# KikeM/romtime

Hardware: AMD Instinct MI355X
Metric: snapshot-DoF/s for POD build (higher is better)
Workload: dtype f64

## Files before the change

romtime_amd/csrc/symeig.hip:

```cpp
#include "common.h"
#include "wave_ops.h"

namespace {

constexpr int TW_SMALL = 32;
constexpr int SLOT0 = 160;
constexpr int TW_LARGE = 128;
constexpr int LPR = 64;
constexpr int TT = 1024;
static_assert(LPR == 64, "row reductions use the whole-wave DPP sum");
constexpr int NMAX = 1024;
constexpr int VEC_ITERS = 2;

struct TriParams {
  const double* G;
  double* V;
  double* P;
  double* tau;
  double* d;
  double* e;
  int* flags;
  int n;
  int tw;
  int local;
  int spread;
  int xcd;
  long* counters;
};

__device__ __forceinline__ void st_wt(double* p, double v) {
  __hip_atomic_store(p, v, __ATOMIC_RELAXED, __HIP_MEMORY_SCOPE_AGENT);
}
__device__ __forceinline__ void st_xcd(double* p, double v, bool one_xcd) {
  if (one_xcd)
    __hip_atomic_store(p, v, __ATOMIC_RELAXED, __HIP_MEMORY_SCOPE_WORKGROUP);
  else
    st_wt(p, v);
}
__device__ __forceinline__ void st_slot(int* p, int v, bool one_xcd) {
  if (one_xcd)
    __hip_atomic_store(p, v, __ATOMIC_RELAXED, __HIP_MEMORY_SCOPE_WORKGROUP);
  else
    __hip_atomic_store(p, v, __ATOMIC_RELAXED, __HIP_MEMORY_SCOPE_AGENT);
}
__device__ __forceinline__ double ld_wt(const double* p) {
  return __hip_atomic_load(p, __ATOMIC_RELAXED, __HIP_MEMORY_SCOPE_AGENT);
}

__device__ __forceinline__ bool poll_slots(int* slots, int TW, int want, int* err) {
  const int lane = threadIdx.x & 63;
  const unsigned long long t0 = __builtin_amdgcn_s_memrealtime();
  for (;;) {
    int f = want;
    for (int w = lane; w < TW; w += 64) {
      const int g = __hip_atomic_load(&slots[w], __ATOMIC_RELAXED, __HIP_MEMORY_SCOPE_AGENT);
      f = g < f ? g : f;
    }
    if (__builtin_amdgcn_ballot_w64(f < want) == 0) return true;
    __builtin_amdgcn_s_sleep(1);
    if (__hip_atomic_load(err, __ATOMIC_RELAXED, __HIP_MEMORY_SCOPE_AGENT) != 0) return false;
    if (__builtin_amdgcn_s_memrealtime() - t0 > 50000000ull) {
      __hip_atomic_store(err, 1, __ATOMIC_RELAXED, __HIP_MEMORY_SCOPE_AGENT);
      return false;
    }
  }
}

__device__ __forceinline__ double block_sum(double x, double* s_red) {
  x = rtw::wave_sum(x);
  const int wid = threadIdx.x >> 6;
  __syncthreads();
  if ((threadIdx.x & 63) == 0) s_red[wid] = x;
  __syncthreads();
  double t = 0.0;
  for (int w = 0; w < TT / 64; ++w) t += s_red[w];
  return t;
}

template <int NM>
__global__ __launch_bounds__(TT) void symeig_tridiag_kernel(const TriParams p) {
  extern __shared__ __attribute__((aligned(16))) double sm[];
  __shared__ int s_ticket;
  if (p.spread) {
    if (threadIdx.x == 0) {
      const int xcc = (int)(__builtin_amdgcn_s_getreg((4 - 1) << 11 | (0 << 6) | 20) & 15u);
      s_ticket = (xcc == p.xcd) ? __hip_atomic_fetch_add(&p.flags[4], 1, __ATOMIC_RELAXED, __HIP_MEMORY_SCOPE_AGENT) : p.tw;
    }
    __syncthreads();
    if (s_ticket >= p.tw) return;
  }
  const int n = p.n, TW = p.tw, tid = threadIdx.x, wg = p.spread ? s_ticket : blockIdx.x, lane = tid & 63,
            wid = tid >> 6;
  const int RB = (n + TW - 1) / TW;
  const bool local = p.local != 0;
  const int lda = local ? n + 2 : n;
  double* A = sm;
  double* svb = sm + (size_t)RB * lda;
  double* sw = svb + 2 * n;
  double* sl = sw + n;
  double* sP = sl + n;
  __shared__ int s_abort;
  if (threadIdx.x == 0) s_abort = 0;
  constexpr int PER = NM / 64;

  for (int q = tid; q < RB * n; q += TT) {
    const int li = q / n, j = q % n, gi = li * TW + wg;
    A[(size_t)li * lda + j] = (gi < n) ? p.G[(size_t)gi * n + j] : 0.0;
  }
  __syncthreads();
  const int ty = tid / LPR, tx = tid % LPR;
  int hop = 0;

  double* L0 = p.P + (size_t)3 * n;
  __shared__ int s_one;
  if (local) {
    for (int j = tid; j < n; j += TT) sl[j] = A[j];
    if (tid == 0) {
      s_one = 0;
      atomicAdd(reinterpret_cast<unsigned long long*>(&p.counters[RT_CNT_EIG_ONE_XCD]), 1ull);
    }
    __syncthreads();
  } else {
  if (wg == 0)
    for (int j = tid; j < n; j += TT) st_wt(&L0[j], A[j]);
  if (tid == 0)
    __hip_atomic_store(&p.flags[8 + wg], (int)__builtin_amdgcn_s_getreg((4 - 1) << 11 | (0 << 6) | 20) + 1,
                       __ATOMIC_RELAXED, __HIP_MEMORY_SCOPE_AGENT);
  asm volatile("s_waitcnt vmcnt(0)" ::: "memory");
  __syncthreads();
  ++hop;
  if (wid == 0) {
    if (lane == 0) st_slot(&p.flags[SLOT0 + wg], hop, false);
    if (!poll_slots(&p.flags[SLOT0], TW, hop, &p.flags[3]) && lane == 0) s_abort = 1;
  }
  __syncthreads();
  if (s_abort) return;
  for (int j = tid; j < n; j += TT) sl[j] = ld_wt(&L0[j]);
  if (tid == 0) {
    const int mine = __hip_atomic_load(&p.flags[8], __ATOMIC_RELAXED, __HIP_MEMORY_SCOPE_AGENT);
    int same = (p.spread != 0) && (mine > 0);
    for (int w = 1; w < TW; ++w)
      same &= (__hip_atomic_load(&p.flags[8 + w], __ATOMIC_RELAXED, __HIP_MEMORY_SCOPE_AGENT) == mine);
    s_one = same;
    if (wg == 0) atomicAdd(reinterpret_cast<unsigned long long*>(&p.counters[same ? RT_CNT_EIG_ONE_XCD : RT_CNT_EIG_GENERAL_FORM]), 1ull);
  }
  __syncthreads();
  }
  const bool one_xcd = s_one != 0;

  __shared__ double s_tauv[2];
  constexpr bool MERGED = NM > 512;
  auto reflector = [&](const double (&x)[PER], int kk, int j0, int off, double diag) {
    double part = 0.0;
#pragma unroll
    for (int q = 0; q < PER; ++q)
      if (q > 0 || lane > off) part = fma(x[q], x[q], part);
    part = rtw::wave_sum(part);
    const double alpha = rtw::read_lane(x[0], off);
    double tau, beta, scale;
    if (part == 0.0) {
      tau = 0.0; beta = alpha; scale = 0.0;
    } else {
      beta = -copysign(sqrt(alpha * alpha + part), alpha);
      tau = (beta - alpha) / beta;
      scale = 1.0 / (alpha - beta);
    }
    const bool owner = (wg == kk % TW);
    double* svk = svb + (size_t)(kk & 1) * n;
#pragma unroll
    for (int q = 0; q < PER; ++q) {
      const int j = j0 + lane + 64 * q;
      const double vq = (q == 0 && lane == off) ? 1.0 : x[q] * scale;
      if (j < n && (q > 0 || lane >= off)) {
        svk[j] = vq;
        if (owner) p.V[(size_t)kk * n + j] = vq;
      }
    }
    if (lane == 0) {
      s_tauv[kk & 1] = tau;
      if (owner) {
        p.tau[kk] = tau;
        p.d[kk] = diag;
        p.e[kk] = beta;
      }
    }
  };

  if (wid == 0 && n > 2) {
    double x[PER];
#pragma unroll
    for (int q = 0; q < PER; ++q) {
      const int j = 1 + lane + 64 * q;
      x[q] = (j < n) ? sl[j] : 0.0;
    }
    reflector(x, 0, 1, 0, sl[0]);
  }
  __syncthreads();
  for (int k = 0; k + 2 < n; ++k) {
    const double* sv = svb + (size_t)(k & 1) * n;
    if constexpr (!MERGED) {
      if (k > 0) {
        if (wid == 0) {
          double x[PER];
#pragma unroll
          for (int q = 0; q < PER; ++q) {
            const int j = k + 1 + lane + 64 * q;
            x[q] = (j < n) ? sl[j] : 0.0;
          }
          reflector(x, k, k + 1, 0, sl[k]);
        }
        __syncthreads();
      }
    }
    const double tau = s_tauv[k & 1];
    double* Pk = p.P + (size_t)(k & 1) * n;
    double* Lk = p.P + (size_t)(2 + (k & 1)) * n;
    if (local) {
      const int gi = tid >> 3, sub = tid & 7;
      double acc = 0.0;
      if (tau != 0.0 && gi > k && gi < n) {
        const double* row = A + (size_t)gi * lda;
        for (int j = k + 1 + sub; j < n; j += 8) acc = fma(row[j], sv[j], acc);
      }
      acc += __shfl_xor(acc, 1);
      acc += __shfl_xor(acc, 2);
      acc += __shfl_xor(acc, 4);
      if (sub == 0 && tau != 0.0 && gi > k && gi < n) sP[gi] = tau * acc;
    } else
    for (int li = ty; li < RB; li += TT / LPR) {
      const int gi = li * TW + wg;
      if (gi > k && gi < n) {
        const double* row = A + (size_t)li * n;
        if (tau != 0.0) {
          double acc = 0.0;
          for (int j = k + 1 + tx; j < n; j += LPR) acc = fma(row[j], sv[j], acc);
          acc = rtw::wave_sum(acc);
          if (tx == 0) {
            if (local) sP[gi] = tau * acc;
            else st_xcd(&Pk[gi], tau * acc, one_xcd);
          }
        }
        if (gi == k + 1 && !local)
          for (int j = k + 1 + tx; j < n; j += LPR) st_xcd(&Lk[j], row[j], one_xcd);
      }
    }
    if (!local) asm volatile("s_waitcnt vmcnt(0)" ::: "memory");
    __syncthreads();
    ++hop;
    if (wid == 0) {
      if (lane == 0 && !local) st_slot(&p.flags[SLOT0 + wg], hop, one_xcd);
      double v[PER];
#pragma unroll
      for (int q = 0; q < PER; ++q) {
        const int j = k + 1 + lane + 64 * q;
        v[q] = (j < n) ? sv[j] : 0.0;
      }
      if (!local && !poll_slots(&p.flags[SLOT0], TW, hop, &p.flags[3])) {
        if (lane == 0) s_abort = 1;
      } else {
        double pv[PER], x[PER];
        const double* nextrow = A + (size_t)(k + 1) * lda;
#pragma unroll
        for (int q = 0; q < PER; ++q) {
          const int j = k + 1 + lane + 64 * q;
          if (local) {
            x[q] = (j < n) ? nextrow[j] : 0.0;
            pv[q] = (j < n && tau != 0.0) ? sP[j] : 0.0;
          } else {
            x[q] = (j < n) ? ld_wt(&Lk[j]) : 0.0;
            pv[q] = (j < n && tau != 0.0) ? ld_wt(&Pk[j]) : 0.0;
          }
        }
        if (tau != 0.0) {
          double dot = 0.0;
#pragma unroll
          for (int q = 0; q < PER; ++q) dot = fma(pv[q], v[q], dot);
          dot = rtw::wave_sum(dot);
          const double alpha2 = -0.5 * tau * dot;
#pragma unroll
          for (int q = 0; q < PER; ++q) pv[q] = fma(alpha2, v[q], pv[q]);
          const double w1 = rtw::first_lane(pv[0]);
#pragma unroll
          for (int q = 0; q < PER; ++q) {
            const int j = k + 1 + lane + 64 * q;
            x[q] = (j < n) ? x[q] - (pv[q] + w1 * v[q]) : 0.0;
            if (j < n) sw[j] = pv[q];
          }
        }
#pragma unroll
        for (int q = 0; q < PER; ++q) {
          const int j = k + 1 + lane + 64 * q;
          if (j < n) sl[j] = x[q];
        }
        if constexpr (MERGED)
          if (k + 3 < n) reflector(x, k + 1, k + 1, 1, rtw::first_lane(x[0]));
      }
    }
    __syncthreads();
    if (s_abort) return;
    if (tau == 0.0) continue;
    if (local) {
      const int gi = tid >> 3, sub = tid & 7;
      if (gi > k && gi < n) {
        double* row = A + (size_t)gi * lda;
        const double vi = sv[gi], wi = sw[gi];
        for (int j = k + 1 + sub; j < n; j += 8) row[j] -= vi * sw[j] + wi * sv[j];
      }
    } else
    for (int li = ty; li < RB; li += TT / LPR) {
      const int gi = li * TW + wg;
      if (gi > k && gi < n) {
        double* row = A + (size_t)li * n;
        const double vi = sv[gi], wi = sw[gi];
        for (int j = k + 1 + tx; j < n; j += LPR) row[j] -= vi * sw[j] + wi * sv[j];
      }
    }
  }
  __syncthreads();
  if (wg == (n - 2) % TW && tid == 0) {
    p.d[n - 2] = sl[n - 2];
    p.e[n - 2] = sl[n - 1];
  }
  if (wg == (n - 1) % TW && tid == 0) {
    p.d[n - 1] = A[(size_t)((n - 1) / TW) * lda + (n - 1)];
    p.e[n - 1] = 0.0;
  }
}

__device__ __forceinline__ double fast_rcp(double q) {
  const double r = __builtin_amdgcn_rcp(q);
  return fma(fma(-q, r, 1.0), r, r);
}

__device__ __forceinline__ int sturm_count(const double* d, const double* e2, int n, double x, double pivmin) {
  double q = d[0] - x;
  if (fabs(q) < pivmin) q = -pivmin;
  int c = (q < 0.0);
  for (int i = 1; i < n; ++i) {
    q = fma(-e2[i - 1], fast_rcp(q), d[i] - x);
    if (fabs(q) < pivmin) q = -pivmin;
    c += (q < 0.0);
  }
  return c;
}

__global__ void symeig_init_kernel(int* flags, double* tau, int n) {
  for (int i = threadIdx.x; i < SLOT0 + TW_LARGE; i += blockDim.x) flags[i] = 0;
  for (int i = threadIdx.x; i < n; i += blockDim.x) tau[i] = 0.0;
}

constexpr int BIS_NS = 2;
template <int NM>
__global__ __launch_bounds__(256) void symeig_bisect_kernel(const double* __restrict__ d, const double* __restrict__ e,
                                                            int n, int first, int count, double* __restrict__ lam,
                                                            const int* flags, int* status, long* counters) {
  if (blockIdx.x == 0 && threadIdx.x == 0) {
    if (status) *status = flags[3];
    if (flags[3]) atomicAdd(reinterpret_cast<unsigned long long*>(&counters[RT_CNT_EIG_TIMEOUT]), 1ull);
  }
  __shared__ double sd[NM], se2[NM];
  __shared__ int s_first[2][4];
  const int tid = threadIdx.x, lane = tid & 63, wid = tid >> 6, half = wid & 1;
  double glo = 1e300, ghi = -1e300, emax = 0.0;
  for (int i = lane; i < n; i += 64) {
    const double di = d[i], ei = (i + 1 < n) ? e[i] : 0.0, el = (i > 0) ? fabs(e[i - 1]) : 0.0;
    sd[i] = di;
    se2[i] = ei * ei;
    glo = fmin(glo, di - el - fabs(ei));
    ghi = fmax(ghi, di + el + fabs(ei));
    emax = fmax(emax, ei * ei);
  }
  glo = rtw::wave_min(glo);
  ghi = rtw::wave_max(ghi);
  emax = rtw::wave_max(emax);
  __syncthreads();
  const double tn = fmax(fabs(glo), fabs(ghi));
  double lo = glo - 2.2e-16 * tn * n - 1e-300, hi = ghi + 2.2e-16 * tn * n + 1e-300;
  const double pivmin = 2.2250738585072014e-308 * fmax(1.0, emax);
  const int j = first + min(2 * (int)blockIdx.x + (wid >> 1), count - 1);
  const int want = n - j;
  constexpr int NSH = 128 * BIS_NS;
  constexpr int NSEC = NSH + 1;
  for (int pass = 0; pass < 7; ++pass) {
    const double h = (hi - lo) / NSEC;
    const int s0 = BIS_NS * (64 * half + lane);
    const double x0 = lo + h * (s0 + 1), x1 = x0 + h;
    double q0 = sd[0] - x0, q1 = sd[0] - x1;
    if (fabs(q0) < pivmin) q0 = -pivmin;
    if (fabs(q1) < pivmin) q1 = -pivmin;
    int c0 = (q0 < 0.0), c1 = (q1 < 0.0);
    for (int i = 1; i < n; ++i) {
      const double di = sd[i], ei = se2[i - 1];
      q0 = fma(-ei, fast_rcp(q0), di - x0);
      q1 = fma(-ei, fast_rcp(q1), di - x1);
      if (fabs(q0) < pivmin) q0 = -pivmin;
      if (fabs(q1) < pivmin) q1 = -pivmin;
      c0 += (q0 < 0.0); c1 += (q1 < 0.0);
    }
    int first = NSH;
    if (c1 >= want) first = s0 + 1;
    if (c0 >= want) first = s0;
    first = rtw::wave_min_i32(first);
    if (lane == 0) s_first[pass & 1][wid] = first;
    __syncthreads();
    first = min(s_first[pass & 1][wid & 2], s_first[pass & 1][(wid & 2) + 1]);
    if (first == NSH) {
      lo = lo + h * NSH;
    } else {
      hi = lo + h * (first + 1);
      lo = lo + h * first;
    }
  }
  if (lane == 0 && half == 0) lam[j] = 0.5 * (lo + hi);
}

struct VecParams {
  const double* d;
  const double* e;
  const double* lam;
  const double* V;
  const double* tau;
  const double* C;
  double* W;
  int n, k;
};

constexpr int RBK = 4;

template <int NM>
__global__ __launch_bounds__(64) void symeig_wy_kernel(const double* __restrict__ V, int n, double* __restrict__ C) {
  constexpr int PER = NM / 64;
  const int b = blockIdx.x, lane = threadIdx.x, k0 = n - 3 - RBK * b;
  double v[RBK][PER];
#pragma unroll
  for (int u = 0; u < RBK; ++u)
#pragma unroll
    for (int q = 0; q < PER; ++q) {
      const int k = k0 - u, j = lane + 64 * q;
      v[u][q] = (k >= 0 && j > k && j < n) ? V[(size_t)k * n + j] : 0.0;
    }
  int slot = 0;
#pragma unroll
  for (int u = 1; u < RBK; ++u)
#pragma unroll
    for (int w = 0; w < u; ++w) {
      double dot = 0.0;
#pragma unroll
      for (int q = 0; q < PER; ++q) dot = fma(v[u][q], v[w][q], dot);
      dot = rtw::wave_sum(dot);
      if (lane == 0) C[6 * b + slot] = dot;
      ++slot;
    }
}

template <int NM>
__global__ __launch_bounds__(64) void symeig_vectors_kernel(const VecParams p) {
  extern __shared__ __attribute__((aligned(16))) double vsm[];
  double *dd = vsm, *ee = dd + NM, *ra = ee + NM + 8, *ub = ra + NM, *ud = ub + NM, *lm = ud + NM, *z = lm + NM,
         *y = z + NM;
  unsigned char* piv = reinterpret_cast<unsigned char*>(y + NM);
  const int n = p.n, t = blockIdx.x, lane = threadIdx.x;
  const double lambda = p.lam[t];
  double tnorm = 0.0;
  for (int i = lane; i < n; i += 64) {
    dd[i] = p.d[i] - lambda;
    ee[i] = (i + 1 < n) ? p.e[i] : 0.0;
    tnorm = fmax(tnorm, fabs(p.d[i]) + 2.0 * ((i + 1 < n) ? fabs(p.e[i]) : 0.0));
    unsigned s = 1664525u * (unsigned)(i + 1 + 7919 * (t + 1)) + 1013904223u;
    s ^= s >> 15; s *= 2246822519u; s ^= s >> 13;
    z[i] = (double)(s & 0xffffff) / 8388608.0 - 1.0;
  }
  if (lane == 0) ee[n] = 0.0;
  tnorm = rtw::wave_max(tnorm);
  const double tiny = 2.2e-16 * fmax(tnorm, 1e-300);
  __syncthreads();
  if (lane == 0) {
    double ak = dd[0], bk = ee[0];
#pragma unroll 4
    for (int k = 0; k + 1 < n; ++k) {
      const double ck = ee[k], an = dd[k + 1], t2 = ee[k + 1];
      const bool swap = fabs(ck) > fabs(ak);
      double pk = swap ? ck : ak;
      if (!swap && fabs(pk) < tiny) pk = copysign(tiny, pk == 0.0 ? 1.0 : pk);
      const double rp = fast_rcp(pk);
      const double mult = (swap ? ak : ck) * rp;
      ra[k] = rp;
      lm[k] = mult;
      piv[k] = swap ? 1 : 0;
      ub[k] = swap ? an : bk;
      ud[k] = swap ? t2 : 0.0;
      const double nd = swap ? fma(-mult, an, bk) : fma(-mult, bk, an);
      bk = swap ? -mult * t2 : t2;
      ak = nd;
    }
    ra[n - 1] = fast_rcp((fabs(ak) < tiny) ? copysign(tiny, ak == 0.0 ? 1.0 : ak) : ak);
    ub[n - 1] = 0.0;
    ud[n - 1] = 0.0;
  }
  __syncthreads();
  for (int it = 0; it < VEC_ITERS; ++it) {
    double zmax = 0.0;
    if (lane == 0) {
      double cur = z[0];
#pragma unroll 4
      for (int k = 0; k + 1 < n; ++k) {
        const double nxt = z[k + 1], ck = lm[k];
        const bool sw = piv[k] != 0;
        y[k] = sw ? nxt : cur;
        cur = sw ? fma(-ck, nxt, cur) : fma(-ck, cur, nxt);
      }
      y[n - 1] = cur;
      double z1 = 0.0, z2 = 0.0;
#pragma unroll 4
      for (int k = n - 1; k >= 0; --k) {
        const double zk = fma(-ud[k], z2, fma(-ub[k], z1, y[k])) * ra[k];
        z[k] = zk;
        zmax = fmax(zmax, fabs(zk));
        z2 = z1;
        z1 = zk;
      }
    }
    zmax = rtw::first_lane(zmax);
    __syncthreads();
    const double sc = 1.0 / fmax(zmax, 1e-300);
    for (int i = lane; i < n; i += 64) z[i] *= sc;
    __syncthreads();
  }
  double part = 0.0;
  for (int i = lane; i < n; i += 64) part += z[i] * z[i];
  part = rtw::wave_sum(part);
  const double inv = 1.0 / sqrt(part);
  for (int i = lane; i < n; i += 64) z[i] *= inv;
  __syncthreads();
  constexpr int PER = NM / 64;
  double zr[PER], vc[RBK][PER], vn[RBK][PER];
#pragma unroll
  for (int q = 0; q < PER; ++q) {
    const int j = lane + 64 * q;
    zr[q] = (j < n) ? z[j] : 0.0;
  }
  auto fetch = [&](int k, double (&dst)[PER]) {
#pragma unroll
    for (int q = 0; q < PER; ++q) {
      const int j = lane + 64 * q;
      dst[q] = (k >= 0 && j > k && j < n) ? p.V[(size_t)k * n + j] : 0.0;
    }
  };
#pragma unroll
  for (int u = 0; u < RBK; ++u) fetch(n - 3 - u, vc[u]);
  int blk = 0;
  for (int k0 = n - 3; k0 >= 0; k0 -= RBK, ++blk) {
#pragma unroll
    for (int u = 0; u < RBK; ++u) fetch(k0 - RBK - u, vn[u]);
    double tk[RBK], cc[6];
#pragma unroll
    for (int u = 0; u < RBK; ++u) tk[u] = (k0 - u >= 0) ? p.tau[k0 - u] : 0.0;
#pragma unroll
    for (int q = 0; q < 6; ++q) cc[q] = p.C[6 * blk + q];
    double a[RBK];
#pragma unroll
    for (int u = 0; u < RBK; ++u) {
      double dot = 0.0;
#pragma unroll
      for (int q = 0; q < PER; ++q) dot = fma(vc[u][q], zr[q], dot);
      a[u] = dot;
    }
#pragma unroll
    for (int u = 0; u < RBK; ++u) a[u] = rtw::wave_sum(a[u]);
    const double s0 = tk[0] * a[0];
    const double s1 = tk[1] * (a[1] - cc[0] * s0);
    const double s2 = tk[2] * (a[2] - cc[1] * s0 - cc[2] * s1);
    const double s3 = tk[3] * (a[3] - cc[3] * s0 - cc[4] * s1 - cc[5] * s2);
#pragma unroll
    for (int q = 0; q < PER; ++q)
      zr[q] = fma(-s3, vc[3][q], fma(-s2, vc[2][q], fma(-s1, vc[1][q], fma(-s0, vc[0][q], zr[q]))));
#pragma unroll
    for (int u = 0; u < RBK; ++u)
#pragma unroll
      for (int q = 0; q < PER; ++q) vc[u][q] = vn[u][q];
  }
#pragma unroll
  for (int q = 0; q < PER; ++q) {
    const int j = lane + 64 * q;
    if (j < n) z[j] = zr[q];
  }
  __syncthreads();
  for (int i = lane; i < n; i += 64) p.W[(size_t)i * p.k + t] = z[i];
}

}

extern "C" int rt_sym_eig_values(rt_ctx* ctx, const double* G, int64_t n, double* lam, int* status) {
  return rt_sym_eig_values_part(ctx, G, n, 0, n, lam, status);
}

extern "C" int rt_sym_eig_values_part(rt_ctx* ctx, const double* G, int64_t n, int64_t first, int64_t count, double* lam,
                                      int* status) {
  if (!ctx) return RT_ERR_ARG;
  RT_ARG_CHECK(ctx, G && lam && n >= 3 && first >= 0 && count >= 1 && first + count <= n);
  if (n > NMAX) {
    ctx->err = "rt_sym_eig_values: n > 1024 not supported (the matrix must stay resident in the LDS of <= 128 CUs)";
    return RT_ERR_UNSUPPORTED;
  }
  const bool large = n > 512;
  const bool small_team = !large && ctx->num_cus < TW_SMALL && ctx->num_cus >= TW_SMALL / 2;
  int tw = large ? TW_LARGE : (small_team ? TW_SMALL / 2 : TW_SMALL);
  const bool local = n <= 64;
  if (local) tw = 1;
  if (tw > ctx->num_cus) {
    ctx->err = "rt_sym_eig_values: not enough compute units for the cooperative tridiagonalisation";
    return RT_ERR_UNSUPPORTED;
  }
  size_t off = 0;
  auto take = [&off](size_t bytes) { size_t o = off; off += (bytes + 255) / 256 * 256; return o; };
  const size_t oV = take(sizeof(double) * n * n), oP = take(sizeof(double) * 4 * n), oT = take(sizeof(double) * n),
               oD = take(sizeof(double) * n), oE = take(sizeof(double) * n), oF = take(sizeof(int) * (SLOT0 + TW_LARGE));
  void* base = nullptr;
  int rc = rt_scratch2(ctx, off, &base);
  if (rc != RT_OK) return rc;
  char* b8 = static_cast<char*>(base);
  TriParams tp;
  tp.G = G; tp.n = (int)n; tp.tw = tw;
  tp.spread = (!large && !local && ctx->eig_one_xcd && ctx->num_cus / 8 >= tw) ? 1 : 0;
  tp.local = local ? 1 : 0;
  tp.xcd = ctx->eig_xcd & 7;
  tp.V = reinterpret_cast<double*>(b8 + oV); tp.P = reinterpret_cast<double*>(b8 + oP);
  tp.tau = reinterpret_cast<double*>(b8 + oT); tp.d = reinterpret_cast<double*>(b8 + oD);
  tp.e = reinterpret_cast<double*>(b8 + oE); tp.flags = reinterpret_cast<int*>(b8 + oF);
  tp.counters = ctx->dev_counters;
  hipStream_t st = ctx->stream;
  hipLaunchKernelGGL(symeig_init_kernel, dim3(1), dim3(256), 0, st, tp.flags, tp.tau, (int)n);

  const int RB = (int)((n + tw - 1) / tw);
  const size_t lds = sizeof(double) * ((size_t)RB * (local ? n + 2 : n) + 5 * n + 16);
  const bool tiny = n <= 256, tinier = n <= 128;
  RT_TRY(rt_func_lds(ctx, reinterpret_cast<const void*>(&symeig_tridiag_kernel<128>), 150 * 1024));
  RT_TRY(rt_func_lds(ctx, reinterpret_cast<const void*>(&symeig_tridiag_kernel<256>), 150 * 1024));
  RT_TRY(rt_func_lds(ctx, reinterpret_cast<const void*>(&symeig_tridiag_kernel<512>), 150 * 1024));
  RT_TRY(rt_func_lds(ctx, reinterpret_cast<const void*>(&symeig_tridiag_kernel<1024>), 150 * 1024));
  {
    int per_cu = 0;
    if (large)
      RT_HIP_CHECK(ctx, hipOccupancyMaxActiveBlocksPerMultiprocessor(&per_cu, symeig_tridiag_kernel<1024>, TT, lds));
    else if (tinier)
      RT_HIP_CHECK(ctx, hipOccupancyMaxActiveBlocksPerMultiprocessor(&per_cu, symeig_tridiag_kernel<128>, TT, lds));
    else if (tiny)
      RT_HIP_CHECK(ctx, hipOccupancyMaxActiveBlocksPerMultiprocessor(&per_cu, symeig_tridiag_kernel<256>, TT, lds));
    else
      RT_HIP_CHECK(ctx, hipOccupancyMaxActiveBlocksPerMultiprocessor(&per_cu, symeig_tridiag_kernel<512>, TT, lds));
    if ((long)per_cu * ctx->num_cus < tw) {
      ctx->err = "rt_sym_eig_values: the device cannot keep all cooperating workgroups resident";
      return RT_ERR_UNSUPPORTED;
    }
  }
  const dim3 bgrid((unsigned)((count + 1) / 2));
  if (large) {
    hipLaunchKernelGGL(symeig_tridiag_kernel<1024>, dim3(tw), dim3(TT), lds, st, tp);
    RT_HIP_CHECK(ctx, hipGetLastError());
    hipLaunchKernelGGL(symeig_bisect_kernel<1024>, bgrid, dim3(256), 0, st, tp.d, tp.e, (int)n, (int)first, (int)count,
                       lam, tp.flags, status, ctx->dev_counters);
  } else {
    if (tinier)
      hipLaunchKernelGGL(symeig_tridiag_kernel<128>, dim3(tp.spread ? 16 * tw : tw), dim3(TT), lds, st, tp);
    else if (tiny)
      hipLaunchKernelGGL(symeig_tridiag_kernel<256>, dim3(tp.spread ? 16 * tw : tw), dim3(TT), lds, st, tp);
    else
      hipLaunchKernelGGL(symeig_tridiag_kernel<512>, dim3(tp.spread ? 16 * tw : tw), dim3(TT), lds, st, tp);
    RT_HIP_CHECK(ctx, hipGetLastError());
    hipLaunchKernelGGL(symeig_bisect_kernel<512>, bgrid, dim3(256), 0, st, tp.d, tp.e, (int)n, (int)first, (int)count,
                       lam, tp.flags, status, ctx->dev_counters);
  }
  RT_HIP_CHECK(ctx, hipGetLastError());
  ctx->eig.d = tp.d; ctx->eig.e = tp.e; ctx->eig.V = tp.V; ctx->eig.tau = tp.tau; ctx->eig.n = n; ctx->eig.base = base;
  ctx->eig.gen = ctx->scratch2_gen;
  return RT_OK;
}

extern "C" int rt_sym_eig_vectors(rt_ctx* ctx, int64_t n, int64_t k, const double* lam, double* W) {
  if (!ctx) return RT_ERR_ARG;
  RT_ARG_CHECK(ctx, lam && W && k >= 1 && k <= n);
  if (ctx->eig.n != n || ctx->eig.base == nullptr || ctx->eig.base != ctx->scratch2 || ctx->eig.gen != ctx->scratch2_gen) {
    ctx->err = "rt_sym_eig_vectors: must follow rt_sym_eig_values on the same ctx and matrix with no other composite "
               "operator (greedy, projection, sweep) in between";
    return RT_ERR_ARG;
  }
  VecParams vp;
  vp.d = ctx->eig.d; vp.e = ctx->eig.e; vp.lam = lam; vp.V = ctx->eig.V; vp.tau = ctx->eig.tau;
  vp.W = W; vp.n = (int)n; vp.k = (int)k;
  const int nblk = (int)((n - 2 + RBK - 1) / RBK);
  void* cbuf = nullptr;
  int rc = rt_scratch(ctx, sizeof(double) * 6 * (size_t)nblk, &cbuf);
  if (rc != RT_OK) return rc;
  vp.C = static_cast<const double*>(cbuf);
  RT_TRY(rt_func_lds(ctx, reinterpret_cast<const void*>(&symeig_vectors_kernel<128>), 80 * 1024));
  RT_TRY(rt_func_lds(ctx, reinterpret_cast<const void*>(&symeig_vectors_kernel<256>), 80 * 1024));
  RT_TRY(rt_func_lds(ctx, reinterpret_cast<const void*>(&symeig_vectors_kernel<512>), 80 * 1024));
  RT_TRY(rt_func_lds(ctx, reinterpret_cast<const void*>(&symeig_vectors_kernel<1024>), 80 * 1024));
  if (n > 512) {
    const size_t vlds = sizeof(double) * (8 * 1024 + 8) + 1024;
    hipLaunchKernelGGL(symeig_wy_kernel<1024>, dim3((unsigned)nblk), dim3(64), 0, ctx->stream, vp.V, (int)n,
                       static_cast<double*>(cbuf));
    hipLaunchKernelGGL(symeig_vectors_kernel<1024>, dim3((unsigned)k), dim3(64), vlds, ctx->stream, vp);
  } else if (n <= 128) {
    const size_t vlds = sizeof(double) * (8 * 128 + 8) + 128;
    hipLaunchKernelGGL(symeig_wy_kernel<128>, dim3((unsigned)nblk), dim3(64), 0, ctx->stream, vp.V, (int)n,
                       static_cast<double*>(cbuf));
    hipLaunchKernelGGL(symeig_vectors_kernel<128>, dim3((unsigned)k), dim3(64), vlds, ctx->stream, vp);
  } else if (n <= 256) {
    const size_t vlds = sizeof(double) * (8 * 256 + 8) + 256;
    hipLaunchKernelGGL(symeig_wy_kernel<256>, dim3((unsigned)nblk), dim3(64), 0, ctx->stream, vp.V, (int)n,
                       static_cast<double*>(cbuf));
    hipLaunchKernelGGL(symeig_vectors_kernel<256>, dim3((unsigned)k), dim3(64), vlds, ctx->stream, vp);
  } else {
    const size_t vlds = sizeof(double) * (8 * 512 + 8) + 512;
    hipLaunchKernelGGL(symeig_wy_kernel<512>, dim3((unsigned)nblk), dim3(64), 0, ctx->stream, vp.V, (int)n,
                       static_cast<double*>(cbuf));
    hipLaunchKernelGGL(symeig_vectors_kernel<512>, dim3((unsigned)k), dim3(64), vlds, ctx->stream, vp);
  }
  RT_HIP_CHECK(ctx, hipGetLastError());
  return RT_OK;
}
```

romtime_amd/pipeline.py:

```python
from __future__ import annotations

import collections
import ctypes as C
import os
import weakref

import numpy as np
import torch

from . import _lib, ops, pod

_p = C.c_void_p


SMALL_SET = 150_000_000
_STREAMS: dict = {}
_STREAMS_PID: list = []
_OPEN_RUNS = weakref.WeakSet()


def shutdown():
    import gc

    if not _STREAMS:
        return
    if _STREAMS_PID and _STREAMS_PID[0] != os.getpid():
        _STREAMS.clear()
        return
    try:
        for gen in list(_OPEN_RUNS):
            gen.close()
        torch.cuda.synchronize()
        gc.collect()
        torch.cuda.empty_cache()
        lib = _lib.load()
        _lib.Context.unbind_streams()
        for st in list(_STREAMS.values()):
            lib.rt_stream_destroy(_p(st.cuda_stream))
    finally:
        _STREAMS.clear()


def _masked_stream(lib, dev, first, count):
    key = (dev, first, count)
    if key not in _STREAMS:
        h = _p()
        rc = lib.rt_stream_create_cu_range(dev, first, count, C.byref(h))
        if rc != 0:
            raise _lib.RomtimeHipError(f"rt_stream_create_cu_range({first}, {count}) failed ({rc})")
        _STREAMS[key] = torch.cuda.ExternalStream(h.value, device=torch.device("cuda", dev))
        _STREAMS_PID[:] = [os.getpid()]
    return _STREAMS[key]


import atexit

atexit.register(shutdown)


class PodPipeline:
    def __init__(self, eig_cus_per_xcd: int = 4, device=None, group=None, eig_first_cu: int = 0, gram_range=None,
                 small_set=None, gram_pace: bool = False):
        self.small_set = SMALL_SET if small_set is None else int(small_set)
        if not torch.cuda.is_available():
            raise _lib.RomtimeHipError("no MI355X visible: romtime_amd's hot path runs on the GPU only")
        self.device = torch.device("cuda", torch.cuda.current_device() if device is None else device)
        dev = self.device.index
        lib = _lib.load()
        self.lib = lib
        per_xcd = torch.cuda.get_device_properties(dev).multi_processor_count // 8
        e = int(eig_cus_per_xcd)
        if not (1 <= e < per_xcd):
            raise ValueError(f"eig_cus_per_xcd must be in [1, {per_xcd})")
        g_first, g_count = gram_range if gram_range is not None else (eig_first_cu + e, per_xcd - e - eig_first_cu)
        if eig_first_cu < 0 or g_count < 1 or g_first + g_count > per_xcd or not (eig_first_cu + e <= g_first or g_first + g_count <= eig_first_cu):
            raise ValueError("the CU ranges of the two streams must be disjoint and inside the XCD")
        self.sE = _masked_stream(lib, dev, eig_first_cu, e)
        self.sG = _masked_stream(lib, dev, g_first, g_count)
        self.ctxE, self.ctxG = _lib.Context(dev), _lib.Context(dev)
        self.ctxE.set_option("cu_limit", 8 * e)
        self.ctxE.set_option("eig_one_xcd", 0)
        self.ctxG.set_option("cu_limit", 8 * g_count)
        self.ctxG.set_option("gram_pace", int(bool(gram_pace)))
        self.group = group
        self.group_e, self.world, self.rank = None, 1, 0
        if group is not None:
            import torch.distributed as dist

            if dist.get_world_size(group) > 1 or os.environ.get("ROMTIME_FORCE_COLLECTIVES"):
                self.group_e = dist.new_group(ranks=dist.get_process_group_ranks(group), backend=dist.get_backend(group))
                self.world, self.rank = dist.get_world_size(group), dist.get_rank(group)
        self.sC = torch.cuda.Stream(self.device) if self.group_e is not None else None
        self.sR = self.sE if self.group_e is not None else None
        self.eig_cus = 8 * e
        self.recomputed = 0
        self.gram_kernel_ms = []
        self.last_stage_ms = {}

    def close(self):
        torch.cuda.synchronize(self.device)

    def _gram(self, item):
        X = item["X"]
        n = X.shape[1]
        with self.ctxG.use(self.sG):
            item["t0"] = torch.cuda.Event(enable_timing=True)
            item["t0"].record()
            Gbuf = torch.empty(n * n + 1, dtype=torch.float64, device=X.device)
            item["G"] = ops.gram(X, out=Gbuf[: n * n].view(n, n))
            Gbuf[n * n:].fill_(float(X.shape[0]))
            item["k0"] = torch.cuda.Event(enable_timing=True)
            item["k0"].record()
            item["Gbuf"] = Gbuf
            if self.sR is None:
                if self.group is not None:
                    import torch.distributed as dist

                    dist.all_reduce(Gbuf, op=dist.ReduceOp.SUM, group=self.group)
                item["g"] = torch.cuda.Event(enable_timing=True)
                item["g"].record()
        if self.sR is not None:
            import torch.distributed as dist

            with torch.cuda.stream(self.sR):
                self.sR.wait_event(item["k0"])
                dist.all_reduce(Gbuf, op=dist.ReduceOp.SUM, group=self.group)
                item["g"] = torch.cuda.Event(enable_timing=True)
                item["g"].record()

    def _eig(self, item):
        k, normalize = item["k"], item["normalize"]
        item["owner"] = item["index"] % self.world
        if self.rank != item["owner"]:
            return
        with self.ctxE.use(self.sE):
            self.sE.wait_event(item["g"])
            G = item["G"]
            n = G.shape[0]
            colnorm, flag = ops.gram_scale(G, normalize)
            lam_d, status = ops.sym_eig_values(G)
            Z = ops.sym_eig_vectors(lam_d, k)
            Zs = ops.backproject_weights(Z, lam_d, colnorm if normalize else None)
            item["payload"] = torch.cat([lam_d, colnorm, status.to(torch.float64), flag.to(torch.float64), Zs.reshape(-1)])
            item["_keep"] = (lam_d, status, flag, Z, Zs, colnorm)
            item["ec"] = torch.cuda.Event(enable_timing=True)
            item["ec"].record()

    def _share(self, item):
        n, k = item["G"].shape[0], item["k"]
        st = self.sE if self.group_e is None else self.sC
        with torch.cuda.stream(st):
            if self.group_e is not None:
                import torch.distributed as dist

                if self.rank == item["owner"]:
                    st.wait_event(item["ec"])
                else:
                    item["payload"] = torch.empty(n * (k + 2) + 2, dtype=torch.float64, device=item["G"].device)
                dist.broadcast(item["payload"], src=dist.get_global_rank(self.group_e, item["owner"]), group=self.group_e)
            payload = item["payload"]
            item["colnorm"].copy_(payload[n:2 * n])
            item["Zs"] = payload[2 * n + 2:].view(n, k)
            head = torch.cat([payload[:n], payload[2 * n:2 * n + 2], item["Gbuf"][-1:]])
            item["head"] = torch.empty(head.numel(), dtype=torch.float64).pin_memory()
            item["head"].copy_(head, non_blocking=True)
            item["_keep2"] = head
            item["e"] = torch.cuda.Event(enable_timing=True)
            item["e"].record()

    def _backproject(self, item):
        ctx, st = self.ctxG, self.sG
        with ctx.use(st):
            st.wait_event(item["e"])
            ops.gemm_nn(item["X"], item["Zs"], out=item["Q"])
            item["b"] = torch.cuda.Event(enable_timing=True)
            item["b"].record()

    def _regular(self, item):
        self.recomputed += 1
        self.sE.synchronize()
        return pod.pod_device(item["X"], num=item["num"], normalize=item["normalize"], group=self.group)

    def _finish(self, item):
        if item["direct"]:
            return self._regular(item)
        item["b"].synchronize()
        n, k = item["X"].shape[1], item["k"]
        head = item["head"].numpy()
        lam, status, zero_norm, n_rows = head[:n], int(head[n]), int(head[n + 1]), int(round(head[n + 2]))
        if item["normalize"] and zero_norm:
            raise ValueError("array must not contain infs or NaNs (zero-norm snapshot with normalize=True)")
        s = np.sqrt(np.clip(lam, 0.0, None))
        energy = pod._energy(s)
        gaps = lam[:k] - lam[1:k + 1] if k < n else np.r_[lam[:k - 1] - lam[1:k], lam[k - 1]]
        ok = (status == 0 and s[0] > 0 and s[k - 1] >= pod.TWO_PASS_RATIO * s[0]
              and gaps.min() >= pod.RR_GAP * max(lam[0], 1e-300) and n_rows >= n)
        self.last_stage_ms = dict(gram_kernel_ms=item["t0"].elapsed_time(item["k0"]),
                                  gram_allreduce_ms=item["t0"].elapsed_time(item["g"]),
                                  eig_chain_ms=item["g"].elapsed_time(item["e"]),
                                  gram_start_to_basis_ms=item["t0"].elapsed_time(item["b"]))
        self.gram_kernel_ms.append(self.last_stage_ms["gram_kernel_ms"])
        if not ok:
            return self._regular(item)
        return dict(Q=item["Q"], s=s, energy=energy, VT=None, r=k, passes=1, colnorm=item["colnorm"])

    def run(self, snapshot_sets, num, normalize=True, depth=2):
        if not num:
            raise ValueError("PodPipeline enqueues ahead of the spectrum: it needs `num` (pod.py:51-53)")
        gen = self._run(snapshot_sets, num, normalize, depth)
        _OPEN_RUNS.add(gen)
        return gen

    def _run(self, snapshot_sets, num, normalize, depth):
        main = torch.cuda.current_stream(self.device)
        flight = collections.deque()
        it = iter(snapshot_sets)
        self._admitted = 0
        depth = max(depth, self.world + 1)

        def after_producer():
            ready = torch.cuda.Event()
            ready.record(main)
            for st in (self.sG, self.sE, self.sC):
                if st is not None:
                    st.wait_event(ready)

        materialised = isinstance(snapshot_sets, (list, tuple))
        if materialised:
            after_producer()

        def admit():
            try:
                X = next(it)
            except StopIteration:
                return None
            if X.dim() != 2 or not X.is_cuda or X.dtype != torch.float64:
                raise _lib.RomtimeHipError("PodPipeline takes 2-D float64 CUDA tensors")
            item = dict(X=X, num=num, k=int(min(num, X.shape[1])), normalize=bool(normalize), index=self._admitted)
            self._admitted += 1
            n = X.shape[1]
            rows = X.shape[0] * self.world
            item["direct"] = not (3 <= n <= 512) or rows * n < self.small_set
            if not item["direct"]:
                item["Q"] = torch.empty((X.shape[0], item["k"]), dtype=torch.float64, device=X.device)
                item["colnorm"] = torch.empty(n, dtype=torch.float64, device=X.device)
                if not materialised:
                    after_producer()
                self._gram(item)
                self._eig(item)
            return item

        pending = collections.deque()
        for _ in range(self.world):
            item = admit()
            if item is None:
                break
            pending.append(item)
        while pending:
            cur = pending.popleft()
            if not cur["direct"]:
                self._share(cur)
            nxt = admit()
            if nxt is not None:
                pending.append(nxt)
            if not cur["direct"]:
                self._backproject(cur)
            flight.append(cur)
            while len(flight) > depth or (not pending and flight):
                yield self._finish(flight.popleft())
        done = torch.cuda.Event()
        done.record(self.sG)
        main.wait_event(done)
        done2 = torch.cuda.Event()
        done2.record(self.sE)
        main.wait_event(done2)
        if self.sC is not None:
            done3 = torch.cuda.Event()
            done3.record(self.sC)
            main.wait_event(done3)

    def map(self, snapshot_sets, num, normalize=True, depth=2):
        return list(self.run(snapshot_sets, num, normalize=normalize, depth=depth))


class PodLanes:

    def __init__(self, lanes: int = 8, device=None):
        if not torch.cuda.is_available():
            raise _lib.RomtimeHipError("no MI355X visible: romtime_amd's hot path runs on the GPU only")
        if not (1 <= int(lanes) <= 8):
            raise ValueError("lanes must be 1 .. 8 (one per XCD)")
        self.device = torch.device("cuda", torch.cuda.current_device() if device is None else device)
        self.ctx, self.streams = [], []
        for lane in range(int(lanes)):
            c = _lib.Context(self.device.index)
            c.set_option("eig_xcd", lane)
            self.ctx.append(c)
            self.streams.append(torch.cuda.Stream(self.device))
        self.recomputed = 0

    def close(self):
        torch.cuda.synchronize(self.device)

    def _enqueue(self, item, lane):
        X, k, normalize = item["X"], item["k"], item["normalize"]
        n = X.shape[1]
        with self.ctx[lane].use(self.streams[lane]):
            Q, lam_d, status2, colnorm, keep = ops.pod_enqueue(X, k, normalize)
            head = torch.cat([lam_d, status2.to(torch.float64)])
            item["head"] = torch.empty(n + 2, dtype=torch.float64).pin_memory()
            item["head"].copy_(head, non_blocking=True)
            item["Q"], item["colnorm"] = Q, colnorm
            item["_keep"] = (keep, head, lam_d, status2)
            item["done"] = torch.cuda.Event()
            item["done"].record()

    def _regular(self, item):
        self.recomputed += 1
        xcd = int(_lib.Context.current().options.get("eig_xcd", 0))
        if xcd < len(self.streams):
            self.streams[xcd].synchronize()
        return pod.pod_device(item["X"], num=item["num"], tol=item["tol"], normalize=item["normalize"])

    def _finish(self, item):
        if item["direct"]:
            return self._regular(item)
        item["done"].synchronize()
        n, k = item["X"].shape[1], item["k"]
        head = item["head"].numpy()
        lam, status, zero_norm = head[:n], int(head[n]), int(head[n + 1])
        if item["normalize"] and zero_norm:
            raise ValueError("array must not contain infs or NaNs (zero-norm snapshot with normalize=True)")
        s = np.sqrt(np.clip(lam, 0.0, None))
        energy = pod._energy(s)
        r = pod.truncation_rank(s, energy, num=item["num"], tol=item["tol"])
        if status != 0 or not (1 <= r <= k) or not s[0] > 0 or item["X"].shape[0] < n:
            return self._regular(item)
        gaps = lam[:r] - lam[1:r + 1] if r < n else np.r_[lam[:r - 1] - lam[1:r], lam[r - 1]]
        if s[r - 1] < pod.TWO_PASS_RATIO * s[0] or gaps.min() < pod.RR_GAP * max(lam[0], 1e-300):
            return self._regular(item)
        Q = item["Q"] if r == k else item["Q"][:, :r]
        for t in (item["Q"], item["colnorm"]):
            t.record_stream(torch.cuda.current_stream(self.device))
        return dict(Q=Q, s=s, energy=energy, VT=None, r=r, passes=1, colnorm=item["colnorm"])

    def run(self, snapshot_sets, num=None, normalize=True, tol=None, cap=64):
        main = torch.cuda.current_stream(self.device)
        it = iter(snapshot_sets)
        pending = collections.deque()
        admitted = 0
        materialised = isinstance(snapshot_sets, (list, tuple))
        if materialised:
            ready = torch.cuda.Event()
            ready.record(main)
            for st in self.streams:
                st.wait_event(ready)

        def admit():
            nonlocal admitted
            try:
                X = next(it)
            except StopIteration:
                return False
            if X.dim() != 2 or not X.is_cuda or X.dtype != torch.float64:
                raise _lib.RomtimeHipError("PodLanes takes 2-D float64 CUDA tensors")
            n = X.shape[1]
            k = int(min(num, n)) if (num and not tol) else int(min(cap, n))
            item = dict(X=X, num=num, tol=tol, k=k, normalize=bool(normalize), direct=not (3 <= n <= 512))
            if not item["direct"]:
                lane = admitted % len(self.streams)
                if not materialised:
                    ready = torch.cuda.Event()
                    ready.record(main)
                    self.streams[lane].wait_event(ready)
                self._enqueue(item, lane)
            admitted += 1
            pending.append(item)
            return True

        for _ in range(len(self.streams)):
            if not admit():
                break
        while pending:
            out = self._finish(pending.popleft())
            admit()
            yield out
        done = torch.cuda.Event()
        for st in self.streams:
            done.record(st)
            main.wait_event(done)

    def map(self, snapshot_sets, num=None, normalize=True, tol=None, cap=64):
        return list(self.run(snapshot_sets, num=num, normalize=normalize, tol=tol, cap=cap))


class PodWorkers:

    def __init__(self, workers: int = 8, device=None):
        import concurrent.futures
        import queue

        if not torch.cuda.is_available():
            raise _lib.RomtimeHipError("no MI355X visible: romtime_amd's hot path runs on the GPU only")
        if not (1 <= int(workers) <= 8):
            raise ValueError("workers must be 1 .. 8 (one eigensolver team per XCD)")
        self.device = torch.device("cuda", torch.cuda.current_device() if device is None else device)
        self.workers = int(workers)
        ids = queue.Queue()
        for i in range(self.workers):
            ids.put(i)
        self._tls = __import__("threading").local()
        dev = self.device

        def init():
            torch.cuda.set_device(dev)
            self._tls.index = ids.get()
            self._tls.stream = torch.cuda.Stream(dev)
            with torch.cuda.stream(self._tls.stream):
                ctx = _lib.Context.current()
                ctx.set_option("eig_xcd", self._tls.index)

        self.pool = concurrent.futures.ThreadPoolExecutor(max_workers=self.workers, initializer=init,
                                                          thread_name_prefix="romtime-pod")

    def _job(self, X, ready, kwargs):
        st = self._tls.stream
        with torch.cuda.stream(st):
            st.wait_event(ready)
            n = X.shape[1]
            if 3 <= n <= 1024 and X.numel() < SMALL_SET:
                Q, s, energy, levels = ops.pod_orth(X, num=kwargs["num"], tol=kwargs["tol"], normalize=kwargs["normalize"])
                if 2 * Q.shape[1] < Q.stride(0):
                    Q = Q.contiguous()
                out = dict(Q=Q, s=s, energy=energy, VT=None, r=int(Q.shape[1]), passes=1 if levels <= 1 else "deflate",
                           levels=levels, colnorm=None)
            else:
                out = pod.pod_device(X, **kwargs)
            done = torch.cuda.Event()
            done.record(st)
        return out, done

    def run(self, snapshot_sets, num=None, tol=None, normalize=True):
        main = torch.cuda.current_stream(self.device)
        kwargs = dict(num=num, tol=tol, normalize=bool(normalize))
        pending = collections.deque()
        it = iter(snapshot_sets)

        def admit():
            try:
                X = next(it)
            except StopIteration:
                return False
            if X.dim() != 2 or not X.is_cuda or X.dtype != torch.float64:
                raise _lib.RomtimeHipError("PodWorkers takes 2-D float64 CUDA tensors")
            ready = torch.cuda.Event()
            ready.record(main)
            pending.append((X, self.pool.submit(self._job, X, ready, kwargs)))
            return True

        for _ in range(self.workers):
            if not admit():
                break
        while pending:
            X, fut = pending.popleft()
            out, done = fut.result()
            main.wait_event(done)
            for t in (out["Q"], out.get("colnorm")):
                if isinstance(t, torch.Tensor) and t.is_cuda:
                    t.record_stream(main)
            admit()
            yield out

    def map(self, snapshot_sets, num=None, tol=None, normalize=True):
        return list(self.run(snapshot_sets, num=num, tol=tol, normalize=normalize))

    def close(self):
        self.pool.shutdown(wait=True)
```

Measured before the change: 91.13 billion.

## Add narrow bisection kernel and deeper lookahead admission in POD pipeline

Adds a bisection eigenvalue kernel that gives each eigenvalue a 16-lane group instead of half a block, using a two-round coarse/fine shift search. It is selected when the eigenvalue count is large relative to the CU count, so more eigenvalues run at once. Separately, the Python pipeline now admits up to four snapshot sets ahead, limited by a memory cap. It also runs the share step right after the eig step when there are no collectives, so gram and eig work for later sets can overlap backprojection. The cost is more device memory held in flight and more reasoning about ordering between streams.

Result: slower. 88.29 billion (-3.1%).

```diff
diff --git a/romtime_amd/csrc/symeig.hip b/romtime_amd/csrc/symeig.hip
--- a/romtime_amd/csrc/symeig.hip
+++ b/romtime_amd/csrc/symeig.hip
@@ -414,6 +414,76 @@
   if (lane == 0 && half == 0) lam[j] = 0.5 * (lo + hi);
 }
 
+constexpr int BIS_LPE = 16;
+static_assert(BIS_LPE * BIS_LPE == 128 * BIS_NS, "two rounds of BIS_LPE shifts cover one pass of the wide form");
+
+template <int NM>
+__global__ __launch_bounds__(256) void symeig_bisect_narrow_kernel(const double* __restrict__ d,
+                                                                   const double* __restrict__ e, int n, int first,
+                                                                   int count, double* __restrict__ lam, const int* flags,
+                                                                   int* status, long* counters) {
+  if (blockIdx.x == 0 && threadIdx.x == 0) {
+    if (status) *status = flags[3];
+    if (flags[3]) atomicAdd(reinterpret_cast<unsigned long long*>(&counters[RT_CNT_EIG_TIMEOUT]), 1ull);
+  }
+  __shared__ double sd[NM], se2[NM];
+  const int tid = threadIdx.x, lane = tid & 63, wid = tid >> 6;
+  constexpr int EPW = 64 / BIS_LPE;
+  const int grp = lane / BIS_LPE, sub = lane % BIS_LPE;
+  double glo = 1e300, ghi = -1e300, emax = 0.0;
+  for (int i = lane; i < n; i += 64) {
+    const double di = d[i], ei = (i + 1 < n) ? e[i] : 0.0, el = (i > 0) ? fabs(e[i - 1]) : 0.0;
+    sd[i] = di;
+    se2[i] = ei * ei;
+    glo = fmin(glo, di - el - fabs(ei));
+    ghi = fmax(ghi, di + el + fabs(ei));
+    emax = fmax(emax, ei * ei);
+  }
+  glo = rtw::wave_min(glo);
+  ghi = rtw::wave_max(ghi);
+  emax = rtw::wave_max(emax);
+  __syncthreads();
+  const double tn = fmax(fabs(glo), fabs(ghi));
+  double lo = glo - 2.2e-16 * tn * n - 1e-300, hi = ghi + 2.2e-16 * tn * n + 1e-300;
+  const double pivmin = 2.2250738585072014e-308 * fmax(1.0, emax);
+  const int slot = (4 * (int)blockIdx.x + wid) * EPW + grp;
+  const int j = first + min(slot, count - 1);
+  const int want = n - j;
+  constexpr int NSH = 128 * BIS_NS;
+  constexpr int NSEC = NSH + 1;
+  auto first_reached = [&](double h, int s) {
+    const double xe = lo + h * ((s & ~1) + 1);
+    const double x = (s & 1) ? xe + h : xe;
+    double q = sd[0] - x;
+    if (fabs(q) < pivmin) q = -pivmin;
+    int c = (q < 0.0);
+#pragma unroll 8
+    for (int i = 1; i < n; ++i) {
+      q = fma(-se2[i - 1], fast_rcp(q), sd[i] - x);
+      if (fabs(q) < pivmin) q = -pivmin;
+      c += (q < 0.0);
+    }
+    const unsigned long long reached = __builtin_amdgcn_ballot_w64(c >= want);
+    const unsigned mine = (unsigned)(reached >> (grp * BIS_LPE)) & ((1u << BIS_LPE) - 1u);
+    return mine ? __builtin_ctz(mine) : BIS_LPE;
+  };
+  for (int pass = 0; pass < 7; ++pass) {
+    const double h = (hi - lo) / NSEC;
+    const int coarse = first_reached(h, BIS_LPE * sub + BIS_LPE - 1);
+    const int fine = first_reached(h, BIS_LPE * min(coarse, BIS_LPE - 1) + sub);
+    if (coarse == BIS_LPE) {
+      lo = lo + h * NSH;
+    } else {
+      const int f = BIS_LPE * coarse + min(fine, BIS_LPE - 1);
+      hi = lo + h * (f + 1);
+      lo = lo + h * f;
+    }
+  }
+  if (sub == 0 && slot < count) lam[j] = 0.5 * (lo + hi);
+}
+
+static bool bisect_narrow(int64_t count, int num_cus) { return 2 * count > 8 * (int64_t)num_cus; }
+
 struct VecParams {
   const double* d;
   const double* e;
@@ -654,11 +724,18 @@
     }
   }
   const dim3 bgrid((unsigned)((count + 1) / 2));
+  const bool narrow = bisect_narrow(count, ctx->num_cus);
+  constexpr int NARROW_EPB = 4 * 64 / BIS_LPE;
+  const dim3 ngrid((unsigned)((count + NARROW_EPB - 1) / NARROW_EPB));
   if (large) {
     hipLaunchKernelGGL(symeig_tridiag_kernel<1024>, dim3(tw), dim3(TT), lds, st, tp);
     RT_HIP_CHECK(ctx, hipGetLastError());
-    hipLaunchKernelGGL(symeig_bisect_kernel<1024>, bgrid, dim3(256), 0, st, tp.d, tp.e, (int)n, (int)first, (int)count,
-                       lam, tp.flags, status, ctx->dev_counters);
+    if (narrow)
+      hipLaunchKernelGGL(symeig_bisect_narrow_kernel<1024>, ngrid, dim3(256), 0, st, tp.d, tp.e, (int)n,
+                         (int)first, (int)count, lam, tp.flags, status, ctx->dev_counters);
+    else
+      hipLaunchKernelGGL(symeig_bisect_kernel<1024>, bgrid, dim3(256), 0, st, tp.d, tp.e, (int)n, (int)first, (int)count,
+                         lam, tp.flags, status, ctx->dev_counters);
   } else {
     if (tinier)
       hipLaunchKernelGGL(symeig_tridiag_kernel<128>, dim3(tp.spread ? 16 * tw : tw), dim3(TT), lds, st, tp);
@@ -667,8 +744,12 @@
     else
       hipLaunchKernelGGL(symeig_tridiag_kernel<512>, dim3(tp.spread ? 16 * tw : tw), dim3(TT), lds, st, tp);
     RT_HIP_CHECK(ctx, hipGetLastError());
-    hipLaunchKernelGGL(symeig_bisect_kernel<512>, bgrid, dim3(256), 0, st, tp.d, tp.e, (int)n, (int)first, (int)count,
-                       lam, tp.flags, status, ctx->dev_counters);
+    if (narrow)
+      hipLaunchKernelGGL(symeig_bisect_narrow_kernel<512>, ngrid, dim3(256), 0, st, tp.d, tp.e, (int)n,
+                         (int)first, (int)count, lam, tp.flags, status, ctx->dev_counters);
+    else
+      hipLaunchKernelGGL(symeig_bisect_kernel<512>, bgrid, dim3(256), 0, st, tp.d, tp.e, (int)n, (int)first, (int)count,
+                         lam, tp.flags, status, ctx->dev_counters);
   }
   RT_HIP_CHECK(ctx, hipGetLastError());
   ctx->eig.d = tp.d; ctx->eig.e = tp.e; ctx->eig.V = tp.V; ctx->eig.tau = tp.tau; ctx->eig.n = n; ctx->eig.base = base;
diff --git a/romtime_amd/pipeline.py b/romtime_amd/pipeline.py
--- a/romtime_amd/pipeline.py
+++ b/romtime_amd/pipeline.py
@@ -14,6 +14,8 @@
 
 
 SMALL_SET = 150_000_000
+DEFAULT_AHEAD = 4
+AHEAD_MEM_FRACTION = 0.25
 _STREAMS: dict = {}
 _STREAMS_PID: list = []
 _OPEN_RUNS = weakref.WeakSet()
@@ -93,6 +95,7 @@
         self.sC = torch.cuda.Stream(self.device) if self.group_e is not None else None
         self.sR = self.sE if self.group_e is not None else None
         self.eig_cus = 8 * e
+        self.ahead_mem_fraction = AHEAD_MEM_FRACTION
         self.recomputed = 0
         self.gram_kernel_ms = []
         self.last_stage_ms = {}
@@ -204,19 +207,24 @@
             return self._regular(item)
         return dict(Q=item["Q"], s=s, energy=energy, VT=None, r=k, passes=1, colnorm=item["colnorm"])
 
-    def run(self, snapshot_sets, num, normalize=True, depth=2):
+    def run(self, snapshot_sets, num, normalize=True, depth=2, ahead=None):
         if not num:
             raise ValueError("PodPipeline enqueues ahead of the spectrum: it needs `num` (pod.py:51-53)")
-        gen = self._run(snapshot_sets, num, normalize, depth)
+        ahead = DEFAULT_AHEAD if ahead is None else int(ahead)
+        if ahead < 1:
+            raise ValueError("ahead must be >= 1")
+        gen = self._run(snapshot_sets, num, normalize, depth, ahead)
         _OPEN_RUNS.add(gen)
         return gen
 
-    def _run(self, snapshot_sets, num, normalize, depth):
+    def _run(self, snapshot_sets, num, normalize, depth, ahead):
         main = torch.cuda.current_stream(self.device)
         flight = collections.deque()
         it = iter(snapshot_sets)
         self._admitted = 0
         depth = max(depth, self.world + 1)
+        ahead = max(ahead, self.world)
+        mem_cap = self.ahead_mem_fraction * torch.cuda.get_device_properties(self.device).total_memory
 
         def after_producer():
             ready = torch.cuda.Event()
@@ -237,6 +245,7 @@
             if X.dim() != 2 or not X.is_cuda or X.dtype != torch.float64:
                 raise _lib.RomtimeHipError("PodPipeline takes 2-D float64 CUDA tensors")
             item = dict(X=X, num=num, k=int(min(num, X.shape[1])), normalize=bool(normalize), index=self._admitted)
+            item["bytes"] = 8 * X.shape[0] * (X.shape[1] + item["k"])
             self._admitted += 1
             n = X.shape[1]
             rows = X.shape[0] * self.world
@@ -248,26 +257,41 @@
                     after_producer()
                 self._gram(item)
                 self._eig(item)
+                if self.group_e is None:
+                    self._share(item)
             return item
 
         pending = collections.deque()
-        for _ in range(self.world):
-            item = admit()
-            if item is None:
-                break
-            pending.append(item)
+        last_bytes = 0
+        exhausted = False
+
+        def fill():
+            nonlocal last_bytes, exhausted
+            while not exhausted and len(pending) < ahead:
+                if len(pending) >= self.world:
+                    alive = sum(i["bytes"] for i in pending) + sum(i["bytes"] for i in flight)
+                    if alive + last_bytes > mem_cap:
+                        break
+                item = admit()
+                if item is None:
+                    exhausted = True
+                    break
+                last_bytes = item["bytes"]
+                pending.append(item)
+
+        fill()
         while pending:
             cur = pending.popleft()
-            if not cur["direct"]:
+            if not cur["direct"] and self.group_e is not None:
                 self._share(cur)
-            nxt = admit()
-            if nxt is not None:
-                pending.append(nxt)
+            while len(flight) >= depth:
+                yield self._finish(flight.popleft())
+            fill()
             if not cur["direct"]:
                 self._backproject(cur)
             flight.append(cur)
-            while len(flight) > depth or (not pending and flight):
-                yield self._finish(flight.popleft())
+        while flight:
+            yield self._finish(flight.popleft())
         done = torch.cuda.Event()
         done.record(self.sG)
         main.wait_event(done)
@@ -279,8 +303,8 @@
             done3.record(self.sC)
             main.wait_event(done3)
 
-    def map(self, snapshot_sets, num, normalize=True, depth=2):
-        return list(self.run(snapshot_sets, num, normalize=normalize, depth=depth))
+    def map(self, snapshot_sets, num, normalize=True, depth=2, ahead=None):
+        return list(self.run(snapshot_sets, num, normalize=normalize, depth=depth, ahead=ahead))
 
 
 class PodLanes:
```
